# jaidevshriram/loma-nerf

Measured on AMD Instinct MI355X. Metric: ray-samples/sec fwd+bwd, 4096 rays×64 samples, 1/2/4/8 MI355X, higher is better.
Workload: dtype f32; 1 GPU; cfg3: 4096 rays x 64 samples per GPU, PE F=5, MLP 33->256x7->4, fp32; rays_per_gpu=4096, samples=64, layers=8, width=256, parallelism=dp1, optimizer=adam lr 0.0005 on device (train_nerf.py:133-161), in the step, input=rays: sampling, dists and positional encoding on the GPU

## Files before the change

### loma-nerf_amd/csrc/lnerf_dw16.hip

```cpp
#include "lnerf_internal.h"

namespace lnerf {

namespace {

typedef float fx4 __attribute__((ext_vector_type(4)));
typedef float fx3 __attribute__((ext_vector_type(3)));
typedef float fx16 __attribute__((ext_vector_type(16)));
typedef __bf16 bf8 __attribute__((ext_vector_type(8)));
typedef __bf16 bf4 __attribute__((ext_vector_type(4)));
typedef _Float16 hf8 __attribute__((ext_vector_type(8)));
typedef _Float16 hf4 __attribute__((ext_vector_type(4)));

#ifndef LNERF_DW16_SPLIT_LATE
#define LNERF_DW16_SPLIT_LATE 1
#endif
#ifndef LNERF_DW16_DEPTH
#define LNERF_DW16_DEPTH 3
#endif

#ifndef LNERF_DW16_XROW
#define LNERF_DW16_XROW 1
#endif

#ifndef LNERF_DW16_WAVES
#define LNERF_DW16_WAVES 8
#endif
constexpr int kWavesDw = LNERF_DW16_WAVES;
static_assert(kWavesDw == 16 || kWavesDw == 8 || kWavesDw == 4, "dW workgroups of 16, 8 or 4 waves");
constexpr int kThreads = 64 * kWavesDw;
constexpr int kTileGroups = kWavesDw / 2;
constexpr int kRPO = 8 / kTileGroups;
constexpr int kRounds = 2 * kRPO;
constexpr int kRows = 512;
#ifndef LNERF_DW16_SWZ
#define LNERF_DW16_SWZ 1
#endif
constexpr int kImgRow = kRows * 2 + (LNERF_DW16_SWZ ? 0 : 64);
__host__ __device__ constexpr int swz(int row) { return LNERF_DW16_SWZ ? (0x18140C00 >> (8 * (row & 3))) & 0xFF : 0; }
constexpr int kPlaneBytes = 16 * kImgRow;
constexpr int kX6A24 = 4;
__host__ __device__ constexpr int nplanes(int PL) { return PL == kX6A24 ? 3 : PL; }
__host__ __device__ constexpr bool a24k(int PL) { return PL == kX6A24 || a24_slabs(PL); }
constexpr int kXrowPL = a24_slabs(2) ? kX6A24 : 3;
template <int PL>
constexpr int image_bytes() { return nplanes(PL) * kPlaneBytes; }

struct Dw16Args {
    int kt[kMaxLayers], nt[kMaxLayers];
    const float* act;
    size_t a_off[kMaxLayers];
    const float* grad;
    size_t g_off[kMaxLayers];
    int blocks;
    int splits[kMaxLayers];
    int nl;
    int lid[kMaxLayers];
    int wg_off[kMaxLayers + 1];
    float* dw_part;
    size_t dwp_off[kMaxLayers];
    float* db_part;
    size_t dbp_off[kMaxLayers];
    const unsigned* sexp;
    int* xcount;
    int rpad;
    const int* eshift;
    int L;
    const int* gate;
};

__device__ __forceinline__ int wave_id() { return __builtin_amdgcn_readfirstlane(threadIdx.x >> 6); }

struct RowMap {
    int lane;
    int hstride;
    int rowo;
    int isamp;
    int tile[kRounds];
    bool ok[kRounds];
};

__device__ __forceinline__ RowMap row_map(int kt, int nt) {
    RowMap m;
    const int t = threadIdx.x, u = t & 127;
    m.lane = 4 * u;
    m.hstride = 512;
    m.rowo = 16 * ((t >> 6) & 1) + 4 * (t & 3);
    m.isamp = (t & 63) >> 2;
    const int w2 = wave_id() >> 1;
#pragma unroll
    for (int i = 0; i < kRounds; ++i) {
        const int tl = kTileGroups * (i % kRPO) + w2;
        m.ok[i] = tl < (i < kRPO ? kt : nt);
        m.tile[i] = m.ok[i] ? tl : 0;
    }
    return m;
}

__device__ __forceinline__ int image_row(int i, const RowMap& m) {
    return (i < kRPO ? 0 : 256) + 32 * (kTileGroups * (i % kRPO) + (threadIdx.x >> 7)) + m.rowo;
}

struct Loads {
    fx4 v[kRounds];
    fx3 a24[kRPO];
    unsigned e;
};

__device__ __forceinline__ void sample_shifts(unsigned e, int E, int& ea, int& eg) {
    const int xa = sexp_xa(e), xg = sexp_xg(e);
    const bool zero = xa == -128 || xg == -128, nonfin = xa == kSexpNonFinite;
    const int d = xa + xg - E;
    ea = zero ? (xa < -126 ? 0 : xa) : nonfin ? E - xg : xa - (d >> 1);
    eg = zero ? (xg == -128 ? 0 : xg) : nonfin ? xg : xg - ((d + 1) >> 1);
}

constexpr int kAllRounds = (1 << kRounds) - 1;
template <bool A24>
__device__ __forceinline__ void issue_loads(const float* A, const float* G, int kt, int nt, const RowMap& m,
// ... 477 lines not shown
                ring[(mine + r) % kXrowRing] = base + k * kThreads + tid;
            }
        }
        tail = off;
        __syncthreads();
        const bool last = base + 4 * kThreads >= p1;
        const int ng = last ? (tail - head + 15) / 16 : (tail - head) / 16;
        if (ng > 0) {
            auto pos = [&](int gi) {
                const int at = head + 16 * gi + m.isamp;
                return at < tail ? ring[at % kXrowRing] : -1;
            };
            int pc = pos(0);
            Loads Lc;
            gather_loads<a24k(PX)>(A, G, se, KT, NT, m, pc, Lc);
            for (int gi = 0; gi < ng; ++gi) {
                const int pn = gi + 1 < ng ? pos(gi + 1) : -1;
                Loads Ln;
                if (gi + 1 < ng) gather_loads<a24k(PX)>(A, G, se, KT, NT, m, pn, Ln);
                float sa, sg;
                sample_scales<PX>(Lc.e, E, sa, sg);
                sa = pc < 0 ? 0.0f : sa;
                sg = pc < 0 ? 0.0f : sg;
                const bool marked = a24k(PX) && sexp_xa(Lc.e) == kSexpNonFinite, anym = a24k(PX) && any_marked(marked);
#pragma unroll
                for (int i = 0; i < kRounds; ++i)
                    if (m.ok[i]) write_planes_row<PX>(round_values<PX>(Lc, i, marked, anym), i, lds, sa, sg, m);
                __syncthreads();
                if (active) mma_block<PX, TI, TJ>(lds, a0, g0, acc);
                __syncthreads();
                Lc = Ln;
                pc = pn;
            }
            head = head + 16 * ng < tail ? head + 16 * ng : tail;
        }
    }
    return int2{tail, ntail};
}

template <int PL>
constexpr int dw_image_bytes() {
    constexpr int main = 2 * image_bytes<PL>();
    constexpr int xr = PL == 2 && LNERF_DW16_XROW ? image_bytes<kXrowPL>() + (kXrowRing + 9 * kWavesDw) * 4 : 0;
    return ((main > xr ? main : xr) + 15) / 16 * 16;
}
template <int PL>
constexpr int dw_chunk_hb() {
    constexpr int room = (160 * 1024 - dw_image_bytes<PL>()) / (16 * (int)sizeof(float2)) - kTabPast;
    return (room > 720 ? 720 : room) / 6 * 6;
}
template <int PL>
constexpr int dw_lds_bytes() { return dw_image_bytes<PL>() + (dw_chunk_hb<PL>() + kTabPast) * 16 * (int)sizeof(float2); }

template <int PL, int TI, int TJ>
__device__ __forceinline__ void dw_split(const Dw16Args& a, int l, int sp, unsigned char* lds) {
    const int tid = threadIdx.x, lane = tid & 63, wave = wave_id();
    const int KT = a.kt[l], NT = a.nt[l];
    const int nbg = (NT + TJ - 1) / TJ, nblk = ((KT + TI - 1) / TI) * nbg;
    const bool active = wave < nblk;
    const int a0 = active ? (wave / nbg) * 32 * TI : 0, g0 = active ? (wave % nbg) * 32 * TJ : 0;
    const int hbs = 2 * a.blocks, splits = a.splits[l];
    const int per = (hbs + splits - 1) / splits;
    const int hb0 = min(hbs, sp * per), hb1 = min(hbs, hb0 + per);

    fx16 acc[TI][TJ];
#pragma unroll
    for (int i = 0; i < TI; ++i)
#pragma unroll
        for (int j = 0; j < TJ; ++j) acc[i][j] = fx16{0, 0, 0, 0, 0, 0, 0, 0, 0, 0, 0, 0, 0, 0, 0, 0};
    fx4 dbs[kRPO];
#pragma unroll
    for (int i = 0; i < kRPO; ++i) dbs[i] = fx4{0.0f, 0.0f, 0.0f, 0.0f};

    const float* A = a.act + a.a_off[l];
    const float* G = a.grad + a.g_off[l];
    const RowMap m = row_map(KT, NT);
    const unsigned* se = a.sexp + (size_t)l * a.rpad;
    const int E = a.eshift[l];
    const bool full = KT == 8 && NT == 8;
    float2* tab = (float2*)(lds + dw_image_bytes<PL>());
    bool xany = false;
    for (int c0 = hb0; c0 < hb1; c0 += dw_chunk_hb<PL>()) {
        const int c1 = min(hb1, c0 + dw_chunk_hb<PL>());
        xany |= fill_scales<PL>(tab, se, E, c0, c1);
        const float2* tabt = tab + m.isamp;
#if LNERF_DW16_DEPTH == 2
        Loads L0, L1;
        issue_loads<a24k(PL)>(A, G, KT, NT, m, c0, c1, L0);
        issue_loads<a24k(PL)>(A, G, KT, NT, m, c0 + 1, c1, L1);
#else
        Loads L0, L1, L2;
        issue_loads<a24k(PL)>(A, G, KT, NT, m, c0, c1, L0);
        issue_loads<a24k(PL)>(A, G, KT, NT, m, c0 + 1, c1, L1);
        issue_loads<a24k(PL)>(A, G, KT, NT, m, c0 + 2, c1, L2);
#endif
        __syncthreads();
#pragma unroll
        for (int i = 0; i < kRPO; ++i) dbs[i] += L0.v[kRPO + i];
        write_planes<PL>(L0, lds, decode_scale(tabt[0]), m);
        float2 scn = tabt[16];
        __syncthreads();
#if LNERF_DW16_DEPTH == 2
        if (active && full) hb_loop2<PL, TI, TJ, true, true>(A, G, tabt, KT, NT, m, c0, c1, a0, g0, acc, L0, L1, dbs, lds, scn);
        else if (active) hb_loop2<PL, TI, TJ, true, false>(A, G, tabt, KT, NT, m, c0, c1, a0, g0, acc, L0, L1, dbs, lds, scn);
        else if (full) hb_loop2<PL, TI, TJ, false, true>(A, G, tabt, KT, NT, m, c0, c1, a0, g0, acc, L0, L1, dbs, lds, scn);
        else hb_loop2<PL, TI, TJ, false, false>(A, G, tabt, KT, NT, m, c0, c1, a0, g0, acc, L0, L1, dbs, lds, scn);
#else
        if (active && full) hb_loop3<PL, TI, TJ, true, true>(A, G, tabt, KT, NT, m, c0, c1, a0, g0, acc, L0, L1, L2, dbs, lds, scn);
        else if (active) hb_loop3<PL, TI, TJ, true, false>(A, G, tabt, KT, NT, m, c0, c1, a0, g0, acc, L0, L1, L2, dbs, lds, scn);
        else if (full) hb_loop3<PL, TI, TJ, false, true>(A, G, tabt, KT, NT, m, c0, c1, a0, g0, acc, L0, L1, L2, dbs, lds, scn);
        else hb_loop3<PL, TI, TJ, false, false>(A, G, tabt, KT, NT, m, c0, c1, a0, g0, acc, L0, L1, L2, dbs, lds, scn);
#endif
    }

    if constexpr (PL == 2 && LNERF_DW16_XROW) {
        const int2 nx = xrow_pass<TI, TJ>(A, G, se, KT, NT, m, hb0, hb1, a0, g0, active, acc, lds, E, xany);
        if (threadIdx.x == 0 && a.xcount) {
            a.xcount[2 * blockIdx.x] = nx.x;
            a.xcount[2 * blockIdx.x + 1] = nx.y;
        }
    } else {
        if (threadIdx.x == 0 && a.xcount) a.xcount[2 * blockIdx.x] = a.xcount[2 * blockIdx.x + 1] = 0;
    }

    if (active) {
        const int ncol = NT * 32, h = lane >> 5;
        float* part = a.dw_part + a.dwp_off[l] + (size_t)sp * (KT * 32) * ncol;
#pragma unroll
        for (int i = 0; i < TI; ++i)
#pragma unroll
            for (int j = 0; j < TJ; ++j) {
                const int kb = a0 + 32 * i, jb = g0 + 32 * j;
                if (kb < KT * 32 && jb < ncol) {
#pragma unroll
                    for (int r = 0; r < 16; ++r) {
                        const int k = kb + (r & 3) + 8 * (r >> 2) + 4 * h;
                        part[(size_t)k * ncol + jb + (lane & 31)] =
                            __builtin_ldexpf(acc[i][j][r], -E);
                    }
                }
            }
    }
    float* red = (float*)lds;
    __syncthreads();
#pragma unroll
    for (int i = 0; i < kRPO; ++i)
#pragma unroll
        for (int j = 0; j < 4; ++j) red[(image_row(kRPO + i, m) - 256 + j) * 16 + m.isamp] = dbs[i][j];
    __syncthreads();
    if (tid < NT * 32) {
        const float* q = red + tid * 16;
        float s0 = 0.0f;
#pragma unroll
        for (int n = 0; n < 16; ++n) s0 += q[n];
        a.db_part[a.dbp_off[l] + (size_t)sp * NT * 32 + tid] = s0;
    }
}

__host__ __device__ __forceinline__ int dw_shape(int kt, int nt) {
    auto fits = [&](int ti, int tj) { return ((kt + ti - 1) / ti) * ((nt + tj - 1) / tj) <= kWavesDw; };
    if (kWavesDw == 8) {
        if (fits(1, 1)) return 0;
        if (fits(1, 2)) return 1;
        return 2;
    }
    if (kWavesDw == 16) {
        if (fits(1, 1)) return 0;
        if (fits(1, 2)) return 1;
        if (fits(2, 1)) return 3;
        return 4;
    }
    if (fits(1, 1)) return 0;
    if (fits(2, 1)) return 3;
    if (fits(1, 2)) return 1;
    if (fits(2, 2)) return 4;
    return 5;
}

template <int PL>
__global__ void __launch_bounds__(kThreads, 1) __attribute__((amdgpu_waves_per_eu(kWavesDw / 4, kWavesDw / 4)))
dw16_kernel(Dw16Args a) {
    __shared__ __attribute__((aligned(256))) unsigned char lds[dw_lds_bytes<PL>()];
    if (a.gate && *a.gate == 0) return;
    int li = 0;
    while (li + 1 < a.nl && (int)blockIdx.x >= a.wg_off[li + 1]) ++li;
    const int l = a.lid[li], sp = blockIdx.x - a.wg_off[li];
    if constexpr (kWavesDw == 8) {
        switch (dw_shape(a.kt[l], a.nt[l])) {
            case 0: dw_split<PL, 1, 1>(a, l, sp, lds); break;
            case 1: dw_split<PL, 1, 2>(a, l, sp, lds); break;
            default: dw_split<PL, 2, 4>(a, l, sp, lds); break;
        }
    } else if constexpr (kWavesDw == 16) {
        switch (dw_shape(a.kt[l], a.nt[l])) {
            case 0: dw_split<PL, 1, 1>(a, l, sp, lds); break;
            case 1: dw_split<PL, 1, 2>(a, l, sp, lds); break;
            case 3: dw_split<PL, 2, 1>(a, l, sp, lds); break;
            default: dw_split<PL, 2, 2>(a, l, sp, lds); break;
        }
    } else {
        switch (dw_shape(a.kt[l], a.nt[l])) {
            case 0: dw_split<PL, 1, 1>(a, l, sp, lds); break;
            case 3: dw_split<PL, 2, 1>(a, l, sp, lds); break;
            case 1: dw_split<PL, 1, 2>(a, l, sp, lds); break;
            case 4: dw_split<PL, 2, 2>(a, l, sp, lds); break;
            default: dw_split<PL, 4, 4>(a, l, sp, lds); break;
        }
    }
}

__global__ void __launch_bounds__(1024) k1_reduce_kernel(const int* __restrict__ epart, int n,
                                                         int* __restrict__ eshift, int nl,
                                                         const float* __restrict__ loss_part, int nwg,
                                                         float* total, float* out_loss, const int* gate) {
    __shared__ float red[1024];
    if (gate && *gate == 0) return;
    const int t = threadIdx.x;
    if ((int)blockIdx.x < nl) {
        const int* q = epart + (size_t)blockIdx.x * n;
        int m = 1 << 20;
        for (int i = t; i < n; i += 1024) m = min(m, q[i]);
        for (int o = 32; o > 0; o >>= 1) m = min(m, __shfl_xor(m, o));
        int* ired = (int*)red;
        if ((t & 63) == 0) ired[t >> 6] = m;
        __syncthreads();
        if (t == 0) {
            int r = ired[0];
            for (int w = 1; w < 16; ++w) r = min(r, ired[w]);
            eshift[blockIdx.x] = r == (1 << 20) ? 0 : r;
        }
        return;
    }
    float s = 0.0f;
    if (t < 256)
        for (int i = t; i < nwg; i += 256) s += loss_part[i];
    red[t] = s;
    __syncthreads();
    for (int w = 128; w > 0; w >>= 1) {
        if (t < w) red[t] = red[t] + red[t + w];
        __syncthreads();
    }
    if (t == 0) {
        *total = red[0];
        if (out_loss) *out_loss = red[0];
    }
}

}

unsigned dw16_build_knobs() {
    return (LNERF_DW16_SPLIT_LATE != 1 ? kKnobDwSplitLate : 0u) | (LNERF_DW16_AHEAD != 1 ? kKnobDwAhead : 0u) | (LNERF_DW16_DEPTH != 3 ? kKnobDwDepth : 0u) |
           (LNERF_DW16_SWZ != 1 ? kKnobDwSwz : 0u) | (LNERF_A24 != 1 ? kKnobA24 : 0u) |
           (LNERF_DW16_XROW != 1 ? kKnobDwXrow : 0u) |
           (LNERF_DW16_WAVES != 8 || !LNERF_DW16_PMAJOR ? kKnobDwWaves : 0u);
}

void dw16_launch(const FusedPlan& p, hipStream_t s) {
    Dw16Args a{};
    for (int l = 0; l < p.L; ++l) {
        a.kt[l] = p.kt[l];
        a.nt[l] = p.nt[l];
        a.a_off[l] = (l == 0) ? p.x_off : p.act_off[l - 1];
        a.g_off[l] = p.grad_off[l];
        a.splits[l] = p.dw_splits[l];
        a.dwp_off[l] = p.dwp_off[l];
        a.dbp_off[l] = p.dbp_off[l];
        a.lid[l] = l;
        a.wg_off[l] = p.dw_split_off[l];
    }
    a.wg_off[p.L] = p.dw_grid;
    a.nl = p.L;
    a.act = p.act;
    a.grad = p.grad;
    a.blocks = p.blocks;
    a.dw_part = p.dw_part;
    a.db_part = p.db_part;
    a.sexp = p.sexp;
    a.xcount = p.xcount;
    a.rpad = p.num_wg * p.tile;
    a.eshift = p.dw_shift;
    a.L = p.L;
    a.gate = p.gate;
    if (p.gate) a.xcount = nullptr;
    static_assert(sizeof(Dw16Args) <= 4096, "kernel arguments");
    if (p.x6 == 2) dw16_kernel<2><<<p.dw_grid, kThreads, 0, s>>>(a);
    else if (p.x6 == 3) dw16_kernel<3><<<p.dw_grid, kThreads, 0, s>>>(a);
    else dw16_kernel<1><<<p.dw_grid, kThreads, 0, s>>>(a);
}

void k1_reduce_launch(const FusedPlan& p, float* out_loss, hipStream_t s) {
    k1_reduce_kernel<<<p.L + 1, 1024, 0, s>>>(p.epart, p.num_wg * (p.tile / 16), p.dw_shift, p.L, p.loss_part,
                                              p.num_wg, p.loss_total, out_loss, p.gate);
}

}
```

### loma-nerf_amd/csrc/lnerf_fused.hip

```cpp
#include "lnerf_internal.h"

#include <stdio.h>

namespace lnerf {

namespace {

constexpr int kTileSamples = 128;

__global__ void __launch_bounds__(256) loss_reduce_kernel(const float* __restrict__ part, int n,
                                                          float* total, float* out_loss) {
    __shared__ float red[256];
    const int t = threadIdx.x;
    float s = 0.0f;
    for (int i = t; i < n; i += 256) s += part[i];
    red[t] = s;
    __syncthreads();
    for (int w = 128; w > 0; w >>= 1) {
        if (t < w) red[t] = red[t] + red[t + w];
        __syncthreads();
    }
    if (t == 0) {
        *total = red[0];
        if (out_loss) *out_loss = red[0];
// ... 267 lines not shown
    p.act = take(y.act_total);
    p.ws_floats = off;
}

void fused_plan(FusedPlan& p, const lnerf_mlp& m, const lnerf_batch& b, void* ws_base, int flags, bool train,
                int dw_grid) {
    if (flags & LNERF_K16_W4) {
        if (flags & LNERF_MFMA_BF16X6) marshal::fail("LNERF_K16_W4 does not run the bf16x6 split (its ring needs 96 KiB)");
        if (b.samples > 64) marshal::fail("LNERF_K16_W4 needs samples <= 64 (whole rays in a 64-sample tile)");
        fused_plan_tile(p, m, b, ws_base, flags, train, dw_grid, 64);
    } else {
        fused_plan_tile(p, m, b, ws_base, flags, train, dw_grid, kTileSamples);
    }
    p.head_fit = (flags & LNERF_HEAD_FIT) ? 1 : 0;
}

static ReduceArgs reduce_args(const FusedPlan& p, const lnerf_outputs& out, int flags) {
    ReduceArgs ra{};
    ra.L = p.L;
    for (int l = 0; l < p.L; ++l) {
        ra.k[l] = p.k[l];
        ra.n[l] = p.n[l];
        ra.kt[l] = p.kt[l];
        ra.nt[l] = p.nt[l];
        ra.splits[l] = p.dw_splits[l];
        ra.dwp_off[l] = p.dwp_off[l];
        ra.dbp_off[l] = p.dbp_off[l];
    }
    ra.w_k = p.w_k;
    ra.w_n = p.w_n;
    ra.dw_part = p.dw_part;
    ra.db_part = p.db_part;
    ra.d_ws = out.d_ws;
    ra.d_bs = out.d_bs;
    ra.scale = (flags & LNERF_SEED_LOSS) ? p.loss_total : nullptr;
    ra.accumulate = (flags & LNERF_ACCUMULATE) ? 1 : 0;
    return ra;
}

void fused_train_step(const FusedPlan& p, const float* ws, const float* bs, const lnerf_batch& b, float seed,
                      int flags, const lnerf_outputs& out, hipStream_t s, hipEvent_t* ev, const FusedPlan* px,
                      float* d_input) {
    const bool seed_loss = (flags & LNERF_SEED_LOSS) != 0;
    auto mark = [&](int i) {
        if (ev) (void)hipEventRecord(ev[i], s);
    };
    const size_t nred = (size_t)p.L * p.w_k * p.w_n + (size_t)p.L * p.w_n;
    const unsigned rgrid = (unsigned)((nred + 255) / 256);
    mark(0);
    k16_pack(p, ws, bs, s);
    mark(1);
    k16_launch(p, b, seed_loss ? 1.0f : seed, out, true, s);
    mark(2);
    k1_reduce_launch(p, out.loss, s);
    mark(3);
    dw16_launch(p, s);
    mark(4);
    if (px && p.guard) {
        k16_launch(*px, b, seed_loss ? 1.0f : seed, out, true, s);
        k1_reduce_launch(*px, out.loss, s);
        dw16_launch(*px, s);
    }
    const ReduceArgs ra = reduce_args(p, out, flags);
    grad_reduce_kernel<<<rgrid, 256, 0, s>>>(ra);
    if (seed_loss) {
        if (out.d_dists) k_scale_by_scalar(out.d_dists, (size_t)p.R, p.loss_total, s);
        if (out.d_target)
            k_scale_by_scalar(out.d_target, (size_t)p.rays * (p.head_fit ? p.n[p.L - 1] : 3), p.loss_total, s);
        if (out.d_x && !d_input) k_scale_by_scalar(out.d_x, (size_t)p.R * p.k[0], p.loss_total, s);
    }
    if (d_input && out.d_x) k_input_grad(b, out.d_x, seed_loss ? p.loss_total : nullptr, d_input, s);
    mark(5);
}

bool fused_render_uses_kr(const FusedPlan& p, int flags) { return !(flags & LNERF_RENDER_K16) && kr_supported(p); }

void fused_render(const FusedPlan& p, const float* ws, const float* bs, const lnerf_batch& b,
                  const lnerf_outputs& out, hipStream_t s, int flags, hipEvent_t* ev) {
    auto mark = [&](int i) {
        if (ev) (void)hipEventRecord(ev[i], s);
    };
    mark(0);
    k16_pack(p, ws, bs, s);
    mark(1);
    int parts = p.num_wg;
    if (fused_render_uses_kr(p, flags)) {
        kr_launch(p, b, out, s);
        parts = kr_num_wg(p);
    } else {
        k16_launch(p, b, 1.0f, out, false, s);
    }
    mark(2);
    if (parts > 4 * 256) {
        const int per = (parts + kLossStage1 - 1) / kLossStage1;
        loss_stage1_kernel<<<kLossStage1, 256, 0, s>>>(p.loss_part, parts, per, p.loss_stage);
        loss_reduce_kernel<<<1, 256, 0, s>>>(p.loss_stage, kLossStage1, p.loss_total, out.loss);
    } else {
        loss_reduce_kernel<<<1, 256, 0, s>>>(p.loss_part, parts, p.loss_total, out.loss);
    }
    mark(3);
    mark(4);
    mark(5);
}

}
```

### loma-nerf_amd/csrc/lnerf_internal.h

```cpp
#pragma once

#include <hip/hip_runtime.h>
#include <stddef.h>
#include <stdint.h>

#include "lnerf.h"
#include "lnerf_marshal.h"

namespace lnerf {

constexpr int kWmaxParts = 32;
constexpr int kHeadCols = 16;
constexpr int kDefaultDwGrid = 512;
__host__ __device__ constexpr int default_dw_grid(long long samples) {
    return samples / 128 >= kDefaultDwGrid ? kDefaultDwGrid : samples / 128 <= 256 ? 256 : (int)(samples / 128);
}
constexpr int kXrowD0 = 12;
constexpr int kXrowLast = 127;
__host__ __device__ constexpr int sexp_xa(unsigned e) { return (int)(signed char)(e & 0xFFu); }
__host__ __device__ constexpr int sexp_xg(unsigned e) { return (int)(signed char)((e >> 16) & 0xFFu); }
__host__ __device__ constexpr int sexp_dmax(unsigned e) { return (int)(signed char)(e >> 24); }

__device__ __forceinline__ int fp16x3_shift(float m) {
    if (!(m > 0.0f) || !(m < __builtin_inff())) return 0;
// ... 127 lines not shown
    int x6;
    int head_fit;
    float* act;
    size_t act_off[kMaxLayers];
    size_t x_off;
    float* grad;
    size_t grad_off[kMaxLayers];
    float* loss_part;
    float* dw_part;
    float* db_part;
    int dw_splits[kMaxLayers];
    int dw_split_off[kMaxLayers];
    size_t dwp_off[kMaxLayers];
    size_t dbp_off[kMaxLayers];
    int dw_grid;
    float* loss_total;
    float* loss_stage;
    int ht16;
    int ks16_f[kMaxLayers], ks16_b[kMaxLayers];
    int to16_f[kMaxLayers], to16_b[kMaxLayers];
    unsigned short* w16;
    unsigned short* w16x;
    size_t w16f_off[kMaxLayers], w16b_off[kMaxLayers];
    float* b16;
    unsigned long long* mask_g;
    int* wexp16;
    int* wmax_part;
    int* hexp16;
    int* dw_shift;
    unsigned* sexp;
    int* xcount;
    int* epart;
    int* guard;
    const int* gate;
    size_t ws_floats;
};

constexpr int kGuardExp = -24;
#ifndef LNERF_GUARD
#define LNERF_GUARD 1
#endif

bool fused_supported(const lnerf_mlp& mlp, int rays, int S, int input_mode, const char** why,
                     bool head_fit = false);
size_t fused_workspace_bytes(const lnerf_mlp& mlp, int rays, int S, bool train = true, int dw_grid = 0);
void fused_plan(FusedPlan& p, const lnerf_mlp& mlp, const lnerf_batch& b, void* ws_base, int flags,
                bool train = true, int dw_grid = 0);
void fused_train_step(const FusedPlan& p, const float* ws, const float* bs, const lnerf_batch& b,
                      float seed, int flags, const lnerf_outputs& out, hipStream_t s,
                      hipEvent_t* ev, const FusedPlan* px = nullptr, float* d_input = nullptr);
void fused_render(const FusedPlan& p, const float* ws, const float* bs, const lnerf_batch& b,
                  const lnerf_outputs& out, hipStream_t s, int flags, hipEvent_t* ev);
bool fused_render_uses_kr(const FusedPlan& p, int flags);
void dw16_launch(const FusedPlan& p, hipStream_t s);
void k1_reduce_launch(const FusedPlan& p, float* out_loss, hipStream_t s);
void k16_pack(const FusedPlan& p, const float* ws, const float* bs, hipStream_t s);
void k16_launch(const FusedPlan& p, const lnerf_batch& b, float seed, const lnerf_outputs& out,
                bool want_grad, hipStream_t s);
void k16_masks_launch(const FusedPlan& p, unsigned char* out, hipStream_t s);
bool kr_supported(const FusedPlan& p);
int kr_num_wg(const FusedPlan& p);
void kr_launch(const FusedPlan& p, const lnerf_batch& b, const lnerf_outputs& out, hipStream_t s);

}
```

### loma-nerf_amd/csrc/lnerf_k16.hip

```cpp
#include "lnerf_composite.h"
#include "lnerf_internal.h"

#include <stddef.h>
#include <stdio.h>

#include <utility>

namespace lnerf {

namespace {

typedef float fx4 __attribute__((ext_vector_type(4)));
typedef __bf16 bf8 __attribute__((ext_vector_type(8)));
typedef _Float16 hf8 __attribute__((ext_vector_type(8)));

constexpr int kWaves = 8;
constexpr int kMaxChunks = 2 * kMaxLayers * 8 + 1;
constexpr int kMaxT = 16;
constexpr int kCompBytes = 2688 * 4;
#ifndef LNERF_K16_FULLDMA
#define LNERF_K16_FULLDMA 1
#endif

template <int PL, int NW = 8, int NG = 1>
// ... 909 lines not shown
                below |= valid[q] && head_floor(act[q][0]) + ex[q] <= kGuardExp;
            }
            sh[q] = unscale(0, ex[q]);
        }
        k16_pass_n<PL, NW, NG>(a, a.ks_b[0], ci, ring, bias_ring, a.to_b[0], act, out, g0s, ex);
#pragma unroll
        for (int q = 0; q < NG; ++q) {
            if (valid[q]) {
#pragma unroll
                for (int o = 0; o < kMaxT; ++o)
                    if (16 * o < a.k0) {
#pragma unroll
                        for (int i = 0; i < 4; ++i) {
                            const int f = 16 * o + 4 * g + i;
                            if (f < a.k0)
                                a.d_x[(size_t)gs[q] * a.k0 + f] =
                                    PL >= 2 ? __builtin_ldexpf(out[q][o][i], sh[q]) : out[q][o][i];
                        }
                    }
            }
        }
    } else {
#pragma unroll
        for (int q = 0; q < NG; ++q) {
            const float xm = sample_max<false>(act[q]);
            store_emin(a, 0, exa[q].get(0), store_sexp(a, 0, 1, xm, dmax[q], lw[q], LW), tail[q], lw[q], LW);
            if (PL == 2 && a.L > 1) below |= valid[q] && gmin[q] + shift_of(xm) <= kGuardExp;
#pragma unroll
            for (int s = 0; s < 8; ++s)
                if (s < a.ks_b[0]) store_slab_step(g0[q] + s * 1024, act[q][2 * s], act[q][2 * s + 1]);
        }
    }
    if (PL == 2 && LNERF_GUARD && a.guard && __builtin_amdgcn_ballot_w64(below) != 0 && lane == 0)
        *a.guard = 1;
#if LNERF_PROF
    PROF_ADD(kPfTail, t_t);
    PROF_ADD(kPfTotal, t_start);
    if (lane == 0) prof_slots()[kPfReal] += __builtin_amdgcn_s_memrealtime() - rt_start;
    if (lane < kPfN) atomicAdd(&g_k16_prof[lane], prof_slots()[lane]);
#endif
}

struct Pack16Args {
    int L;
    int k[kMaxLayers], n[kMaxLayers];
    int ks_f[kMaxLayers], ks_b[kMaxLayers], to_f[kMaxLayers], to_b[kMaxLayers];
    int w_k, w_n, planes;
    const float* W;
    const float* B;
    unsigned short* w16;
    size_t wf_off[kMaxLayers], wb_off[kMaxLayers];
    float* b16;
    int* wexp;
    int* wpart;
    int* hexp;
    int* hpart;
    int* guard_reset;
    unsigned short* w16x;
    const int* gate;
};

__global__ void __launch_bounds__(256) wmax16_kernel(Pack16Args a) {
    const int l = blockIdx.y;
    const float* W = a.W + (size_t)l * a.w_k * a.w_n;
    const int K = a.k[l], N = a.n[l];
    float m = 0.0f;
    for (int k = blockIdx.x; k < K; k += gridDim.x)
        for (int j = threadIdx.x; j < N; j += blockDim.x) m = fmaxf(m, fabsf(W[(size_t)k * a.w_n + j]));
    for (int o = 32; o > 0; o >>= 1) m = fmaxf(m, __shfl_xor(m, o));
    __shared__ float red[4];
    if ((threadIdx.x & 63) == 0) red[threadIdx.x >> 6] = m;
    __syncthreads();
    if (threadIdx.x == 0)
        a.wpart[l * kWmaxParts + blockIdx.x] =
            __float_as_int(fmaxf(fmaxf(red[0], red[1]), fmaxf(red[2], red[3])));
    if (l == a.L - 1 && threadIdx.x < kHeadCols) {
        const int j = threadIdx.x;
        float mc = 0.0f;
        if (j < N)
            for (int k = blockIdx.x; k < K; k += gridDim.x) mc = fmaxf(mc, fabsf(W[(size_t)k * a.w_n + j]));
        a.hpart[blockIdx.x * kHeadCols + j] = __float_as_int(mc);
    }
}


__device__ __forceinline__ int layer_wmax(Pack16Args& a, int l) {
    int mb = 0;
    for (int i = 0; i < kWmaxParts; ++i) mb = max(mb, a.wpart[l * kWmaxParts + i]);
    if (blockIdx.x == 0 && threadIdx.x == 0) a.wexp[l] = mb;
    return mb;
}


__global__ void pack16_kernel(Pack16Args a) {
    if (a.gate && *a.gate == 0) return;
    if (a.guard_reset && blockIdx.x == 0 && blockIdx.y == 0 && threadIdx.x == 0) *a.guard_reset = 0;
    const int l = blockIdx.y;
    const float* W = a.W + (size_t)l * a.w_k * a.w_n;
    const int K = a.k[l], N = a.n[l];
    const int lmax = a.planes == 2 ? layer_wmax(a, l) : 0;
    const int wsh = a.planes == 2 ? wshift_of(lmax) : 0;
    const bool head = a.planes == 2 && l == a.L - 1;
    __shared__ int hsh[kHeadCols];
    if (head) {
        if (threadIdx.x < kHeadCols) {
            int mb = 0;
            for (int i = 0; i < kWmaxParts; ++i) mb = max(mb, a.hpart[i * kHeadCols + threadIdx.x]);
            hsh[threadIdx.x] = head_col_shift(mb, lmax);
            if (blockIdx.x == 0) a.hexp[threadIdx.x] = mb;
        }
        __syncthreads();
    }
    const size_t nf = (size_t)a.ks_f[l] * a.to_f[l] * 512, nb = (size_t)a.ks_b[l] * a.to_b[l] * 512;
    for (size_t e = blockIdx.x * (size_t)blockDim.x + threadIdx.x; e < nf + nb + 256;
         e += (size_t)gridDim.x * blockDim.x) {
        if (e >= nf + nb) {
            const int f = (int)(e - nf - nb);
            a.b16[(size_t)l * 256 + f] = f < N ? a.B[(size_t)l * a.w_n + f] : 0.0f;
            continue;
        }
        const bool fwd = e < nf;
        size_t x = fwd ? e : e - nf;
        const int to = fwd ? a.to_f[l] : a.to_b[l];
        const int j = x & 7; x >>= 3;
        const int ln = x & 63; x >>= 6;
        const int o = (int)(x % to); x /= to;
        const int s = (int)x;
        const int f = phi(s, ln >> 4, j), m = 16 * o + (ln & 15);
        const int kk = fwd ? f : m, jj = fwd ? m : f;
        const float w = (kk < K && jj < N) ? W[(size_t)kk * a.w_n + jj] : 0.0f;
        unsigned short* dst = a.w16 + (fwd ? a.wf_off[l] : a.wb_off[l]) +
                              ((size_t)(s * to + o) * a.planes) * 512 + ln * 8 + j;
        if (a.planes == 2) {
            _Float16 h, lo;
            split_h(__builtin_ldexpf(w, head && jj < kHeadCols ? hsh[jj] : wsh), h, lo);
            dst[0] = __builtin_bit_cast(unsigned short, h);
            dst[512] = __builtin_bit_cast(unsigned short, lo);
            if (a.w16x) {
                unsigned short* dx = a.w16x + (fwd ? a.wf_off[l] : a.wb_off[l]) + ((size_t)(s * to + o) * 3) * 512 +
                                     ln * 8 + j;
                __bf16 xh, xm, xl;
                split_x(w, xh, xm, xl);
                dx[0] = __builtin_bit_cast(unsigned short, xh);
                dx[512] = __builtin_bit_cast(unsigned short, xm);
                dx[1024] = __builtin_bit_cast(unsigned short, xl);
            }
            continue;
        }
        __bf16 h, mi, lo;
        split_x(w, h, mi, lo);
        dst[0] = __builtin_bit_cast(unsigned short, h);
        if (a.planes == 3) {
            dst[512] = __builtin_bit_cast(unsigned short, mi);
            dst[1024] = __builtin_bit_cast(unsigned short, lo);
        }
    }
}

__global__ void k16_masks_kernel(const unsigned long long* __restrict__ mask_g, int L1, int R, int tile_samples,
                                 int nw, unsigned char* __restrict__ out) {
    const size_t idx = (size_t)blockIdx.x * blockDim.x + threadIdx.x;
    if (idx >= (size_t)L1 * R * 32) return;
    const int b = (int)(idx & 31);
    const size_t lr = idx >> 5;
    const int l = (int)(lr / R), r = (int)(lr % R);
    const int wg = r / tile_samples, ls = r % tile_samples, wave = ls >> 4, n = ls & 15;
    const int o = b >> 1, g0 = 2 * (b & 1);
    const unsigned long long* w = mask_g + ((size_t)(wg * L1 + l) * nw + wave) * 64;
    const unsigned lo = (unsigned)(w[g0 * 16 + n] >> (4 * o)) & 0xFu;
    const unsigned hi = (unsigned)(w[(g0 + 1) * 16 + n] >> (4 * o)) & 0xFu;
    out[idx] = (unsigned char)(lo | (hi << 4));
}

}

unsigned k16_build_knobs() {
    return (LNERF_K16_FULLDMA != 1 ? kKnobK16FullDma : 0u) | (LNERF_K16_KDIST != 2 ? kKnobK16KDist : 0u) |
           (LNERF_K16_SPLIT_AT != 2 ? kKnobK16SplitAt : 0u) | (LNERF_K16_SCHED != 1 ? kKnobK16Sched : 0u) |
           (LNERF_K16_PRIO != 0 ? kKnobK16Prio : 0u) | (LNERF_K16_SPREAD != 1 ? kKnobK16Spread : 0u) |
           (LNERF_PROF != 0 ? kKnobProf : 0u) | (LNERF_A24 != 1 ? kKnobA24 : 0u) |
           (LNERF_K16_PIN != 2 ? kKnobK16Pin : 0u) | (LNERF_K16_FDSRC != 1 ? kKnobK16FdSrc : 0u) |
           (LNERF_K16_ONECHUNK != 1 ? kKnobK16OneChunk : 0u) | (LNERF_K16_WAVECOMP != 1 ? kKnobK16WaveComp : 0u) |
           (LNERF_K16_EPIFMA != 1 ? kKnobK16EpiFma : 0u) | (LNERF_K16_G2 != 0 ? kKnobK16G2 : 0u) |
           (LNERF_PE_DOUBLING != 1 ? kKnobPeDoubling : 0u) | (LNERF_GUARD != 1 ? kKnobGuard : 0u)
#ifdef LNERF_K16_ONLY_16_2
           | kKnobK16Only
#endif
        ;
}

void k16_masks_launch(const FusedPlan& p, unsigned char* out, hipStream_t s) {
    const size_t n = (size_t)(p.L - 1) * p.R * 32;
    if (n == 0) return;
    k16_masks_kernel<<<(unsigned)((n + 255) / 256), 256, 0, s>>>(p.mask_g, p.L - 1, p.R, p.rays_per_wg * p.S,
                                                                 p.tile / 16, out);
}

void k16_pack(const FusedPlan& p, const float* ws, const float* bs, hipStream_t s) {
    Pack16Args a{};
    a.L = p.L;
    for (int l = 0; l < p.L; ++l) {
        a.k[l] = p.k[l];
        a.n[l] = p.n[l];
        a.ks_f[l] = p.ks16_f[l];
        a.ks_b[l] = p.ks16_b[l];
        a.to_f[l] = p.to16_f[l];
        a.to_b[l] = p.to16_b[l];
        a.wf_off[l] = p.w16f_off[l];
        a.wb_off[l] = p.w16b_off[l];
    }
    a.w_k = p.w_k;
    a.w_n = p.w_n;
    a.planes = p.x6;
    a.W = ws;
    a.B = bs;
    a.w16 = p.w16;
    a.b16 = p.b16;
    a.wexp = p.wexp16;
    a.wpart = p.wmax_part;
    a.hexp = p.hexp16;
    a.hpart = p.wmax_part + (size_t)kMaxLayers * kWmaxParts;
    a.guard_reset = p.guard;
    a.gate = p.gate;
    a.w16x = p.x6 == 2 ? p.w16x : nullptr;
    if (a.planes == 2) wmax16_kernel<<<dim3(kWmaxParts, p.L), 256, 0, s>>>(a);
    size_t nmax = 0;
    for (int l = 0; l < p.L; ++l) {
        const size_t nel = ((size_t)a.ks_f[l] * a.to_f[l] + (size_t)a.ks_b[l] * a.to_b[l]) * 512 + 256;
        nmax = nel > nmax ? nel : nmax;
    }
    pack16_kernel<<<dim3((unsigned)((nmax + 255) / 256), p.L), 256, 0, s>>>(a);
}

void k16_launch(const FusedPlan& p, const lnerf_batch& b, float seed, const lnerf_outputs& out,
                bool want_grad, hipStream_t s) {
    K16Args a{};
    a.L = p.L;
    for (int l = 0; l < p.L; ++l) {
        a.ks_f[l] = p.ks16_f[l];
        a.ks_b[l] = p.ks16_b[l];
        a.to_f[l] = p.to16_f[l];
        a.to_b[l] = p.to16_b[l];
        a.kt[l] = p.kt[l];
        a.nt[l] = p.nt[l];
        a.wf_off[l] = p.w16f_off[l];
        a.wb_off[l] = p.w16b_off[l];
        a.act_off[l] = p.act_off[l];
        a.grad_off[l] = p.grad_off[l];
    }
    a.k0 = p.k[0];
    a.w16 = p.w16;
    a.b16 = p.b16;
    a.mask_g = p.mask_g;
    a.act = p.act;
    a.x_off = p.x_off;
    a.grad = p.grad;
    a.rays = p.rays;
    a.S = p.S;
    a.rpw = p.rays_per_wg;
    a.R = p.R;
    a.input_mode = b.input_mode;
    a.F = b.num_freqs;
    a.near_t = b.near_t;
    a.far_t = b.far_t;
    a.x = b.x;
    a.dists = b.input_mode == LNERF_INPUT_RAYS ? nullptr : b.dists;
    a.target = b.target;
    a.loss_part = p.loss_part;
    a.acc_color = out.acc_color;
    a.d_dists = want_grad ? out.d_dists : nullptr;
    a.d_target = want_grad ? out.d_target : nullptr;
    a.d_x = want_grad ? out.d_x : nullptr;
    a.seed = seed;
    a.want_grad = want_grad ? 1 : 0;
    a.head_fit = p.head_fit;
    a.nout = p.n[p.L - 1];
    a.planes = p.x6;
    a.wexp = p.wexp16;
    a.hexp = p.hexp16;
    a.sexp = (unsigned char*)p.sexp;
    a.rpad = p.num_wg * p.tile;
    a.epart = p.epart;
    a.guard = want_grad && p.x6 == 2 ? p.guard : nullptr;
    a.gate = p.gate;
// ... 61 lines not shown
```

Measured before the change: 117.7 million ray-samples/s.

## Fold exponent/loss reduction into dW kernel and merge weight max-scan into pack kernel

Removes the separate k1_reduce launch: each dW workgroup now computes its layer's exponent shift from the per-workgroup partials itself, and block 0 sums the batch loss before starting its dW work. The wmax16 pre-pass is also removed: pack16 now scans each layer's absolute max redundantly in every one of its 32 workgroups, and each thread packs a full 8-element row with vectorised 16-byte stores. The aim is fewer kernel launches and less per-launch overhead in the step. The cost is redundant reduction work in every dW and pack workgroup, plus extra serial loss-reduction work on dW block 0.

```diff
diff --git a/loma-nerf_amd/csrc/lnerf_dw16.hip b/loma-nerf_amd/csrc/lnerf_dw16.hip
--- a/loma-nerf_amd/csrc/lnerf_dw16.hip
+++ b/loma-nerf_amd/csrc/lnerf_dw16.hip
@@ -25,6 +25,9 @@
 
 #ifndef LNERF_DW16_WAVES
 #define LNERF_DW16_WAVES 8
+#endif
+#ifndef LNERF_DW16_LOSS_AT
+#define LNERF_DW16_LOSS_AT 0
 #endif
 constexpr int kWavesDw = LNERF_DW16_WAVES;
 static_assert(kWavesDw == 16 || kWavesDw == 8 || kWavesDw == 4, "dW workgroups of 16, 8 or 4 waves");
@@ -64,7 +67,13 @@
     const unsigned* sexp;
     int* xcount;
     int rpad;
-    const int* eshift;
+    const int* epart;
+    int nepart;
+    int* eshift;
+    const float* loss_part;
+    int nwg;
+    float* loss_total;
+    float* out_loss;
     int L;
     const int* gate;
 };
@@ -648,6 +657,50 @@
 template <int PL>
 constexpr int dw_lds_bytes() { return dw_image_bytes<PL>() + (dw_chunk_hb<PL>() + kTabPast) * 16 * (int)sizeof(float2); }
 
+__device__ __forceinline__ int layer_shift(const int* __restrict__ q, int n, int* red) {
+    typedef int i4 __attribute__((ext_vector_type(4)));
+    const int t = threadIdx.x, n4 = n >> 2;
+    const i4* q4 = (const i4*)q;
+    int m = 1 << 20;
+    for (int i = t; i < n4; i += kThreads) {
+        const i4 v = q4[i];
+        m = min(m, min(min(v[0], v[1]), min(v[2], v[3])));
+    }
+    for (int i = 4 * n4 + t; i < n; i += kThreads) m = min(m, q[i]);
+    for (int o = 32; o > 0; o >>= 1) m = min(m, __shfl_xor(m, o));
+    if ((t & 63) == 0) red[t >> 6] = m;
+    __syncthreads();
+    int r = red[0];
+#pragma unroll
+    for (int w = 1; w < kWavesDw; ++w) r = min(r, red[w]);
+    return __builtin_amdgcn_readfirstlane(r == (1 << 20) ? 0 : r);
+}
+
+__device__ __attribute__((noinline)) int layer_shift_call(const int* __restrict__ q, int n, int* red) {
+    return layer_shift(q, n, red);
+}
+
+__device__ __forceinline__ void batch_loss(const float* __restrict__ part, int n, float* total,
+                                                     float* out_loss, float* red) {
+    const int t = threadIdx.x;
+    if (t < 256) {
+        float s = 0.0f;
+        for (int i = t; i < n; i += 256) s += part[i];
+        red[t] = s;
+    }
+    __syncthreads();
+    for (int w = 128; w > 0; w >>= 1) {
+        if (t < w) red[t] = red[t] + red[t + w];
+        __syncthreads();
+    }
+    if (t == 0) {
+        const float v = red[0];
+        *total = v;
+        if (out_loss) *out_loss = v;
+    }
+    __syncthreads();
+}
+
 template <int PL, int TI, int TJ>
 __device__ __forceinline__ void dw_split(const Dw16Args& a, int l, int sp, unsigned char* lds) {
     const int tid = threadIdx.x, lane = tid & 63, wave = wave_id();
@@ -672,7 +725,14 @@
     const float* G = a.grad + a.g_off[l];
     const RowMap m = row_map(KT, NT);
     const unsigned* se = a.sexp + (size_t)l * a.rpad;
-    const int E = a.eshift[l];
+    int E;
+    if constexpr (PL == 3) {
+        E = layer_shift_call(a.epart + (size_t)l * a.nepart, a.nepart, (int*)lds);
+        asm volatile("s_waitcnt lgkmcnt(0)" ::: "memory");
+    } else {
+        E = layer_shift(a.epart + (size_t)l * a.nepart, a.nepart, (int*)lds);
+    }
+    if (sp == 0 && tid == 0) a.eshift[l] = E;
     const bool full = KT == 8 && NT == 8;
     float2* tab = (float2*)(lds + dw_image_bytes<PL>());
     bool xany = false;
@@ -778,6 +838,7 @@
 dw16_kernel(Dw16Args a) {
     __shared__ __attribute__((aligned(256))) unsigned char lds[dw_lds_bytes<PL>()];
     if (a.gate && *a.gate == 0) return;
+    if (LNERF_DW16_LOSS_AT == 0 && blockIdx.x == 0) batch_loss(a.loss_part, a.nwg, a.loss_total, a.out_loss, (float*)lds);
     int li = 0;
     while (li + 1 < a.nl && (int)blockIdx.x >= a.wg_off[li + 1]) ++li;
     const int l = a.lid[li], sp = blockIdx.x - a.wg_off[li];
@@ -803,42 +864,9 @@
             default: dw_split<PL, 4, 4>(a, l, sp, lds); break;
         }
     }
-}
-
-__global__ void __launch_bounds__(1024) k1_reduce_kernel(const int* __restrict__ epart, int n,
-                                                         int* __restrict__ eshift, int nl,
-                                                         const float* __restrict__ loss_part, int nwg,
-                                                         float* total, float* out_loss, const int* gate) {
-    __shared__ float red[1024];
-    if (gate && *gate == 0) return;
-    const int t = threadIdx.x;
-    if ((int)blockIdx.x < nl) {
-        const int* q = epart + (size_t)blockIdx.x * n;
-        int m = 1 << 20;
-        for (int i = t; i < n; i += 1024) m = min(m, q[i]);
-        for (int o = 32; o > 0; o >>= 1) m = min(m, __shfl_xor(m, o));
-        int* ired = (int*)red;
-        if ((t & 63) == 0) ired[t >> 6] = m;
+    if (LNERF_DW16_LOSS_AT != 0 && blockIdx.x == gridDim.x - 1) {
         __syncthreads();
-        if (t == 0) {
-            int r = ired[0];
-            for (int w = 1; w < 16; ++w) r = min(r, ired[w]);
-            eshift[blockIdx.x] = r == (1 << 20) ? 0 : r;
-        }
-        return;
-    }
-    float s = 0.0f;
-    if (t < 256)
-        for (int i = t; i < nwg; i += 256) s += loss_part[i];
-    red[t] = s;
-    __syncthreads();
-    for (int w = 128; w > 0; w >>= 1) {
-        if (t < w) red[t] = red[t] + red[t + w];
-        __syncthreads();
-    }
-    if (t == 0) {
-        *total = red[0];
-        if (out_loss) *out_loss = red[0];
+        batch_loss(a.loss_part, a.nwg, a.loss_total, a.out_loss, (float*)lds);
     }
 }
 
@@ -848,10 +876,10 @@
     return (LNERF_DW16_SPLIT_LATE != 1 ? kKnobDwSplitLate : 0u) | (LNERF_DW16_AHEAD != 1 ? kKnobDwAhead : 0u) | (LNERF_DW16_DEPTH != 3 ? kKnobDwDepth : 0u) |
            (LNERF_DW16_SWZ != 1 ? kKnobDwSwz : 0u) | (LNERF_A24 != 1 ? kKnobA24 : 0u) |
            (LNERF_DW16_XROW != 1 ? kKnobDwXrow : 0u) |
-           (LNERF_DW16_WAVES != 8 || !LNERF_DW16_PMAJOR ? kKnobDwWaves : 0u);
-}
-
-void dw16_launch(const FusedPlan& p, hipStream_t s) {
+           (LNERF_DW16_WAVES != 8 || !LNERF_DW16_PMAJOR || LNERF_DW16_LOSS_AT != 0 ? kKnobDwWaves : 0u);
+}
+
+void dw16_launch(const FusedPlan& p, float* out_loss, hipStream_t s) {
     Dw16Args a{};
     for (int l = 0; l < p.L; ++l) {
         a.kt[l] = p.kt[l];
@@ -874,7 +902,13 @@
     a.sexp = p.sexp;
     a.xcount = p.xcount;
     a.rpad = p.num_wg * p.tile;
+    a.epart = p.epart;
+    a.nepart = p.num_wg * (p.tile / 16);
     a.eshift = p.dw_shift;
+    a.loss_part = p.loss_part;
+    a.nwg = p.num_wg;
+    a.loss_total = p.loss_total;
+    a.out_loss = out_loss;
     a.L = p.L;
     a.gate = p.gate;
     if (p.gate) a.xcount = nullptr;
@@ -884,9 +918,4 @@
     else dw16_kernel<1><<<p.dw_grid, kThreads, 0, s>>>(a);
 }
 
-void k1_reduce_launch(const FusedPlan& p, float* out_loss, hipStream_t s) {
-    k1_reduce_kernel<<<p.L + 1, 1024, 0, s>>>(p.epart, p.num_wg * (p.tile / 16), p.dw_shift, p.L, p.loss_part,
-                                              p.num_wg, p.loss_total, out_loss, p.gate);
-}
-
-}
+}
diff --git a/loma-nerf_amd/csrc/lnerf_fused.hip b/loma-nerf_amd/csrc/lnerf_fused.hip
--- a/loma-nerf_amd/csrc/lnerf_fused.hip
+++ b/loma-nerf_amd/csrc/lnerf_fused.hip
@@ -343,14 +343,12 @@
     mark(1);
     k16_launch(p, b, seed_loss ? 1.0f : seed, out, true, s);
     mark(2);
-    k1_reduce_launch(p, out.loss, s);
     mark(3);
-    dw16_launch(p, s);
+    dw16_launch(p, out.loss, s);
     mark(4);
     if (px && p.guard) {
         k16_launch(*px, b, seed_loss ? 1.0f : seed, out, true, s);
-        k1_reduce_launch(*px, out.loss, s);
-        dw16_launch(*px, s);
+        dw16_launch(*px, out.loss, s);
     }
     const ReduceArgs ra = reduce_args(p, out, flags);
     grad_reduce_kernel<<<rgrid, 256, 0, s>>>(ra);
diff --git a/loma-nerf_amd/csrc/lnerf_internal.h b/loma-nerf_amd/csrc/lnerf_internal.h
--- a/loma-nerf_amd/csrc/lnerf_internal.h
+++ b/loma-nerf_amd/csrc/lnerf_internal.h
@@ -203,8 +203,7 @@
 void fused_render(const FusedPlan& p, const float* ws, const float* bs, const lnerf_batch& b,
                   const lnerf_outputs& out, hipStream_t s, int flags, hipEvent_t* ev);
 bool fused_render_uses_kr(const FusedPlan& p, int flags);
-void dw16_launch(const FusedPlan& p, hipStream_t s);
-void k1_reduce_launch(const FusedPlan& p, float* out_loss, hipStream_t s);
+void dw16_launch(const FusedPlan& p, float* out_loss, hipStream_t s);
 void k16_pack(const FusedPlan& p, const float* ws, const float* bs, hipStream_t s);
 void k16_launch(const FusedPlan& p, const lnerf_batch& b, float seed, const lnerf_outputs& out,
                 bool want_grad, hipStream_t s);
diff --git a/loma-nerf_amd/csrc/lnerf_k16.hip b/loma-nerf_amd/csrc/lnerf_k16.hip
--- a/loma-nerf_amd/csrc/lnerf_k16.hip
+++ b/loma-nerf_amd/csrc/lnerf_k16.hip
@@ -985,107 +985,152 @@
     size_t wf_off[kMaxLayers], wb_off[kMaxLayers];
     float* b16;
     int* wexp;
-    int* wpart;
     int* hexp;
-    int* hpart;
     int* guard_reset;
     unsigned short* w16x;
     const int* gate;
 };
 
-__global__ void __launch_bounds__(256) wmax16_kernel(Pack16Args a) {
-    const int l = blockIdx.y;
+constexpr int kPackThreads = 512;
+constexpr int kPackWgs = 32;
+
+__device__ __forceinline__ float abs_max4(float m, const fx4& v) {
+    return fmaxf(m, fmaxf(fmaxf(fabsf(v[0]), fabsf(v[1])), fmaxf(fabsf(v[2]), fabsf(v[3]))));
+}
+
+__device__ __forceinline__ float scan_wmax(const float* __restrict__ W, int K, int N, int w_n) {
+    const int t = threadIdx.x;
+    float m = 0.0f;
+    if (w_n % 4 == 0 && N % 4 == 0 && (uintptr_t)W % 16 == 0) {
+        const int nq = N >> 2, tot = K * nq;
+        for (int i0 = t; i0 < tot; i0 += 8 * kPackThreads) {
+            fx4 v[8];
+#pragma unroll
+            for (int u = 0; u < 8; ++u) {
+                const int i = i0 + u * kPackThreads, ic = i < tot ? i : i0;
+                const int k = ic / nq, q = ic - k * nq;
+                v[u] = *(const fx4*)(W + (size_t)k * w_n + 4 * q);
+            }
+#pragma unroll
+            for (int u = 0; u < 8; ++u) m = abs_max4(m, v[u]);
+        }
+    } else {
+        const int tot = K * N;
+        for (int i0 = t; i0 < tot; i0 += 8 * kPackThreads) {
+            float v[8];
+#pragma unroll
+            for (int u = 0; u < 8; ++u) {
+                const int i = i0 + u * kPackThreads, ic = i < tot ? i : i0;
+                const int k = ic / N, j = ic - k * N;
+                v[u] = W[(size_t)k * w_n + j];
+            }
+#pragma unroll
+            for (int u = 0; u < 8; ++u) m = fmaxf(m, fabsf(v[u]));
+        }
+    }
+    return m;
+}
+
+__device__ __forceinline__ void store_row8(unsigned short* dst, const unsigned short (&v)[8]) {
+    typedef unsigned ux4 __attribute__((ext_vector_type(4)));
+    *(ux4*)dst = ux4{v[0] | ((unsigned)v[1] << 16), v[2] | ((unsigned)v[3] << 16), v[4] | ((unsigned)v[5] << 16),
+                     v[6] | ((unsigned)v[7] << 16)};
+}
+
+__global__ void __launch_bounds__(kPackThreads) pack16_kernel(Pack16Args a) {
+    if (a.gate && *a.gate == 0) return;
+    if (a.guard_reset && blockIdx.x == 0 && blockIdx.y == 0 && threadIdx.x == 0) *a.guard_reset = 0;
+    const int l = blockIdx.y, t = threadIdx.x;
     const float* W = a.W + (size_t)l * a.w_k * a.w_n;
     const int K = a.k[l], N = a.n[l];
-    float m = 0.0f;
-    for (int k = blockIdx.x; k < K; k += gridDim.x)
-        for (int j = threadIdx.x; j < N; j += blockDim.x) m = fmaxf(m, fabsf(W[(size_t)k * a.w_n + j]));
-    for (int o = 32; o > 0; o >>= 1) m = fmaxf(m, __shfl_xor(m, o));
-    __shared__ float red[4];
-    if ((threadIdx.x & 63) == 0) red[threadIdx.x >> 6] = m;
-    __syncthreads();
-    if (threadIdx.x == 0)
-        a.wpart[l * kWmaxParts + blockIdx.x] =
-            __float_as_int(fmaxf(fmaxf(red[0], red[1]), fmaxf(red[2], red[3])));
-    if (l == a.L - 1 && threadIdx.x < kHeadCols) {
-        const int j = threadIdx.x;
-        float mc = 0.0f;
-        if (j < N)
-            for (int k = blockIdx.x; k < K; k += gridDim.x) mc = fmaxf(mc, fabsf(W[(size_t)k * a.w_n + j]));
-        a.hpart[blockIdx.x * kHeadCols + j] = __float_as_int(mc);
-    }
-}
-
-
-__device__ __forceinline__ int layer_wmax(Pack16Args& a, int l) {
-    int mb = 0;
-    for (int i = 0; i < kWmaxParts; ++i) mb = max(mb, a.wpart[l * kWmaxParts + i]);
-    if (blockIdx.x == 0 && threadIdx.x == 0) a.wexp[l] = mb;
-    return mb;
-}
-
-
-__global__ void pack16_kernel(Pack16Args a) {
-    if (a.gate && *a.gate == 0) return;
-    if (a.guard_reset && blockIdx.x == 0 && blockIdx.y == 0 && threadIdx.x == 0) *a.guard_reset = 0;
-    const int l = blockIdx.y;
-    const float* W = a.W + (size_t)l * a.w_k * a.w_n;
-    const int K = a.k[l], N = a.n[l];
-    const int lmax = a.planes == 2 ? layer_wmax(a, l) : 0;
+    const bool head = a.planes == 2 && l == a.L - 1;
+    __shared__ float wred[kPackThreads / 64];
+    __shared__ float cred[16][kHeadCols];
+    __shared__ int hsh[kHeadCols];
+    int lmax = 0;
+    if (a.planes == 2) {
+        float m = scan_wmax(W, K, N, a.w_n);
+        for (int o = 32; o > 0; o >>= 1) m = fmaxf(m, __shfl_xor(m, o));
+        if ((t & 63) == 0) wred[t >> 6] = m;
+        if (head && t < 16 * kHeadCols) {
+            const int j = t & (kHeadCols - 1), r = t >> 4;
+            float mc = 0.0f;
+            if (j < N) {
+                float v[16];
+#pragma unroll
+                for (int u = 0; u < 16; ++u) v[u] = W[(size_t)min(r + 16 * u, K - 1) * a.w_n + j];
+#pragma unroll
+                for (int u = 0; u < 16; ++u) mc = fmaxf(mc, fabsf(v[u]));
+            }
+            cred[r][j] = mc;
+        }
+        __syncthreads();
+        float lm = wred[0];
+#pragma unroll
+        for (int w = 1; w < kPackThreads / 64; ++w) lm = fmaxf(lm, wred[w]);
+        lmax = __float_as_int(lm);
+        if (blockIdx.x == 0 && t == 0) a.wexp[l] = lmax;
+        if (head) {
+            if (t < kHeadCols) {
+                float mc = 0.0f;
+#pragma unroll
+                for (int r = 0; r < 16; ++r) mc = fmaxf(mc, cred[r][t]);
+                const int mb = __float_as_int(mc);
+                hsh[t] = head_col_shift(mb, lmax);
+                if (blockIdx.x == 0) a.hexp[t] = mb;
+            }
+            __syncthreads();
+        }
+    }
     const int wsh = a.planes == 2 ? wshift_of(lmax) : 0;
-    const bool head = a.planes == 2 && l == a.L - 1;
-    __shared__ int hsh[kHeadCols];
-    if (head) {
-        if (threadIdx.x < kHeadCols) {
-            int mb = 0;
-            for (int i = 0; i < kWmaxParts; ++i) mb = max(mb, a.hpart[i * kHeadCols + threadIdx.x]);
-            hsh[threadIdx.x] = head_col_shift(mb, lmax);
-            if (blockIdx.x == 0) a.hexp[threadIdx.x] = mb;
-        }
-        __syncthreads();
-    }
-    const size_t nf = (size_t)a.ks_f[l] * a.to_f[l] * 512, nb = (size_t)a.ks_b[l] * a.to_b[l] * 512;
-    for (size_t e = blockIdx.x * (size_t)blockDim.x + threadIdx.x; e < nf + nb + 256;
-         e += (size_t)gridDim.x * blockDim.x) {
-        if (e >= nf + nb) {
-            const int f = (int)(e - nf - nb);
-            a.b16[(size_t)l * 256 + f] = f < N ? a.B[(size_t)l * a.w_n + f] : 0.0f;
-            continue;
-        }
+    const size_t gt = blockIdx.x * (size_t)kPackThreads + t, gn = (size_t)gridDim.x * kPackThreads;
+    for (size_t f = gt; f < 256; f += gn) a.b16[(size_t)l * 256 + f] = (int)f < N ? a.B[(size_t)l * a.w_n + f] : 0.0f;
+    const size_t nf = (size_t)a.ks_f[l] * a.to_f[l] * 64, nb = (size_t)a.ks_b[l] * a.to_b[l] * 64;
+    for (size_t e = gt; e < nf + nb; e += gn) {
         const bool fwd = e < nf;
         size_t x = fwd ? e : e - nf;
         const int to = fwd ? a.to_f[l] : a.to_b[l];
-        const int j = x & 7; x >>= 3;
         const int ln = x & 63; x >>= 6;
         const int o = (int)(x % to); x /= to;
         const int s = (int)x;
-        const int f = phi(s, ln >> 4, j), m = 16 * o + (ln & 15);
-        const int kk = fwd ? f : m, jj = fwd ? m : f;
-        const float w = (kk < K && jj < N) ? W[(size_t)kk * a.w_n + jj] : 0.0f;
-        unsigned short* dst = a.w16 + (fwd ? a.wf_off[l] : a.wb_off[l]) +
-                              ((size_t)(s * to + o) * a.planes) * 512 + ln * 8 + j;
+        const int m = 16 * o + (ln & 15);
+        float w[8];
+        int sh[8];
+#pragma unroll
+        for (int j = 0; j < 8; ++j) {
+            const int f = phi(s, ln >> 4, j);
+            const int kk = fwd ? f : m, jj = fwd ? m : f;
+            w[j] = (kk < K && jj < N) ? W[(size_t)kk * a.w_n + jj] : 0.0f;
+            sh[j] = head && jj < kHeadCols ? hsh[jj] : wsh;
+        }
+        const size_t lo0 = fwd ? a.wf_off[l] : a.wb_off[l];
+        unsigned short* dst = a.w16 + lo0 + ((size_t)(s * to + o) * a.planes) * 512 + ln * 8;
+        unsigned short p0[8], p1[8], p2[8];
         if (a.planes == 2) {
-            _Float16 h, lo;
-            split_h(__builtin_ldexpf(w, head && jj < kHeadCols ? hsh[jj] : wsh), h, lo);
-            dst[0] = __builtin_bit_cast(unsigned short, h);
-            dst[512] = __builtin_bit_cast(unsigned short, lo);
-            if (a.w16x) {
-                unsigned short* dx = a.w16x + (fwd ? a.wf_off[l] : a.wb_off[l]) + ((size_t)(s * to + o) * 3) * 512 +
-                                     ln * 8 + j;
-                __bf16 xh, xm, xl;
-                split_x(w, xh, xm, xl);
-                dx[0] = __builtin_bit_cast(unsigned short, xh);
-                dx[512] = __builtin_bit_cast(unsigned short, xm);
-                dx[1024] = __builtin_bit_cast(unsigned short, xl);
-            }
-            continue;
-        }
-        __bf16 h, mi, lo;
-        split_x(w, h, mi, lo);
-        dst[0] = __builtin_bit_cast(unsigned short, h);
-        if (a.planes == 3) {
-            dst[512] = __builtin_bit_cast(unsigned short, mi);
-            dst[1024] = __builtin_bit_cast(unsigned short, lo);
+#pragma unroll
+            for (int j = 0; j < 8; ++j) {
+                _Float16 h, lo;
+                split_h(__builtin_ldexpf(w[j], sh[j]), h, lo);
+                p0[j] = __builtin_bit_cast(unsigned short, h);
+                p1[j] = __builtin_bit_cast(unsigned short, lo);
+            }
+            store_row8(dst, p0);
+            store_row8(dst + 512, p1);
+            if (!a.w16x) continue;
+            dst = a.w16x + lo0 + ((size_t)(s * to + o) * 3) * 512 + ln * 8;
+        }
+#pragma unroll
+        for (int j = 0; j < 8; ++j) {
+            __bf16 h, mi, lo;
+            split_x(w[j], h, mi, lo);
+            p0[j] = __builtin_bit_cast(unsigned short, h);
+            p1[j] = __builtin_bit_cast(unsigned short, mi);
+            p2[j] = __builtin_bit_cast(unsigned short, lo);
+        }
+        store_row8(dst, p0);
+        if (a.planes != 1) {
+            store_row8(dst + 512, p1);
+            store_row8(dst + 1024, p2);
         }
     }
 }
@@ -1150,19 +1195,11 @@
     a.w16 = p.w16;
     a.b16 = p.b16;
     a.wexp = p.wexp16;
-    a.wpart = p.wmax_part;
     a.hexp = p.hexp16;
-    a.hpart = p.wmax_part + (size_t)kMaxLayers * kWmaxParts;
     a.guard_reset = p.guard;
     a.gate = p.gate;
     a.w16x = p.x6 == 2 ? p.w16x : nullptr;
-    if (a.planes == 2) wmax16_kernel<<<dim3(kWmaxParts, p.L), 256, 0, s>>>(a);
-    size_t nmax = 0;
-    for (int l = 0; l < p.L; ++l) {
-        const size_t nel = ((size_t)a.ks_f[l] * a.to_f[l] + (size_t)a.ks_b[l] * a.to_b[l]) * 512 + 256;
-        nmax = nel > nmax ? nel : nmax;
-    }
-    pack16_kernel<<<dim3((unsigned)((nmax + 255) / 256), p.L), 256, 0, s>>>(a);
+    pack16_kernel<<<dim3(kPackWgs, p.L), kPackThreads, 0, s>>>(a);
 }
 
 void k16_launch(const FusedPlan& p, const lnerf_batch& b, float seed, const lnerf_outputs& out,
```

After: 117.8 million ray-samples/s, median of 2. About the same (+0.0%).
